# underactuated/HSLabs

Hardware: AMD Instinct MI355X
Metric: batched control-loop steps/sec (hexapod.xml, 18-DoF) at 1/2/4/8 MI355X (higher is better)
Workload: dtype f64

## Files before the change

### hslabs_amd/csrc/hs_limb.h

```cpp

#ifndef HS_LIMB_GROUP
#define HS_LIMB_GROUP HS_FUSED_GROUP
#endif
#ifndef HS_LIMB_WAVES
#define HS_LIMB_WAVES 2
#endif
#ifndef HS_LIMB_WAVES_F32
#define HS_LIMB_WAVES_F32 HS_LIMB_WAVES
#endif

constexpr int LG = 8;
constexpr int LGR = WAVE / LG;

__device__ unsigned long long g_limb_deferred;

template <int NM, bool FORCES = false>
struct LimbLds {
  real g[NM][6];
  real a[6];
  real wd[HS_NMAX];
  real p[FORCES ? NM : 1][3];
};

__device__ inline real grp_get(real v, int src) { return __shfl(v, src); }
// ... 29 lines not shown
  {
    const real cm[3] = {(real)lk.com[0], (real)lk.com[1], (real)lk.com[2]};
    mulp(H, cm, P);
  }
  {
    real R[9];
#pragma unroll
    for (int i = 0; i < 9; i++) R[i] = (real)lk.Rpj[i];
    auto a_rc = [&](int r, int c) { return H(r, 0) * R[c * 3 + 0] + H(r, 1) * R[c * 3 + 1] + H(r, 2) * R[c * 3 + 2]; };
    U[0] = (a_rc(2, 1) - a_rc(1, 2)) / 2;
    U[1] = (a_rc(0, 2) - a_rc(2, 0)) / 2;
    U[2] = (a_rc(1, 0) - a_rc(0, 1)) / 2;
  }
  if (CENTRE) {
#pragma unroll
    for (int i = 0; i < 3; i++) Jp[i] = Jv(i, 3);
#pragma unroll
    for (int i = 0; i < 3; i++) Jz[i] = Jv(i, 2);
    if (kk == 2) {
      const real cp[3] = {(real)lk.cap[0], (real)lk.cap[1], (real)lk.cap[2]};
      mulp(H, cp, fp);
      contact = fp[2] < (real)(T->rcap + 1e-4);
    }
  }
}

__device__ inline void part_dyn(real m, real inv, const real* Pm, const real* P0, const real* Pp, const real* Um,
                                const real* U0, const real* Up, real* f) {
  real vp[3], vm[3], mr[3], wp[3], wm[3], amr[3];
  for (int j = 0; j < 3; j++) {
    vp[j] = Pp[j] - P0[j];
    vp[j] *= inv;
    vm[j] = P0[j] - Pm[j];
    vm[j] *= inv;
    real mp = vp[j] * m, mm = vm[j] * m;
    mr[j] = mp - mm;
    mr[j] *= inv;
    wp[j] = Up[j] - U0[j];
    wp[j] *= inv;
    wm[j] = U0[j] - Um[j];
    wm[j] *= inv;
  }
  for (int j = 0; j < 3; j++) {
    amr[j] = wp[j] - wm[j];
    amr[j] *= inv;
  }
  for (int j = 0; j < 3; j++) {
    f[j] = mr[j];
    f[3 + j] = amr[j];
  }
  opaque_vals<6>(f);
  f[2] += m * real(1);
}

__device__ inline void part_g(const real* P, const real* o, real* f) {
  opaque_vals<6>(f);
  real d[3];
  for (int j = 0; j < 3; j++) d[j] = P[j] - o[j];
  f[3] += d[1] * f[2] - d[2] * f[1];
  f[4] += d[2] * f[0] - d[0] * f[2];
  f[5] += d[0] * f[1] - d[1] * f[0];
  opaque_vals<6>(f);
}

struct BodyS {
  real P[3], U[3];
};
__device__ inline BodyS body_straight(const real* bf, const real* u, real tv) {
  BodyS s;
  for (int i = 0; i < 3; i++) s.P[i] = fma(tv, u[i], bf[i]);
  for (int i = 0; i < 3; i++) s.U[i] = bf[3 + i];
  return s;
}
__device__ inline BodyS body_frame(const A34& A, const real* com) {
  BodyS s;
  mulp(A, com, s.P);
  s.U[0] = (A(2, 1) - A(1, 2)) / 2;
  s.U[1] = (A(0, 2) - A(2, 0)) / 2;
  s.U[2] = (A(1, 0) - A(0, 1)) / 2;
  return s;
}

__device__ __attribute__((always_inline)) inline A34 limb_frame(const hs_topo* T, int L, bool straight, const bool own,
                                                                const RolloutWS& W, int row, const real* u, real tv,
                                                                BodyS& ob) {
  if (straight) {
    if (own) ob = body_straight(W.kf.own[L][0], u, tv);
    return frame_at(load34r(W.kf.J0[L]), u, tv);
  }
  A34 A = load34r(W.ktor[row] + 6);
  const int clen = T->limb_chain_len[L];
  for (int kk = 1; kk < clen; kk++) {
    const int v = T->limb_chain[L][kk];
    A = mul(A, node_pj(T, v));
    if (T->node[v].owner_limb == L) {
      const real com[3] = {(real)T->node[v].com[0], (real)T->node[v].com[1], (real)T->node[v].com[2]};
      ob = body_frame(A, com);
    }
  }
  return mul(A, node_joint_parent(T, T->limb_child[L]));
}

__device__ inline bool sincos_big(real x) { return !(fabs(x) < (real)0x1p20); }
__device__ __attribute__((always_inline)) inline void limb_outer(const hs_topo* T, const hs_link (&LK)[3], const A34& J,
                                                                 const real* ja, real (&P)[3][3], real (&U)[3][3],
                                                                 bool& big) {
  real sq[3], cq[3];
#pragma unroll
  for (int kk = 0; kk < 3; kk++) {
    big |= sincos_big(ja[kk]);
    sincos_k_small(ja[kk], &sq[kk], &cq[kk]);
  }
  A34 Jv = J, H;
  real nul[3];
  bool nc = false;
#pragma unroll
  for (int kk = 0; kk < 3; kk++) fk_link<false>(T, LK[kk], kk, Jv, H, sq[kk], cq[kk], P[kk], U[kk], nul, nul, nul, nc);
}

__device__ __attribute__((always_inline)) inline void contact_block(const real (&Jp)[3][3], const real (&Jz)[3][3],
                                                                    const real (&xt)[3][3], const real* fp, real* Dp6,
                                                                    real* gc) {
  real tD[3][6], tg[3][3];
#pragma unroll
  for (int m = 0; m < 3; m++) {
    const int p = 2 - m;
    real Dp[6] = {0, 0, 0, 0, 0, 0}, g[3] = {0, 0, 0};
    real da[3], va[3][3];
    for (int r = 0; r < 3; r++) da[r] = Jp[p][r] - fp[r];
    cross_rows(da, va);
#pragma unroll
    for (int r = 0; r < 3; r++) {
      const real w2 = Jz[p][r] * Jz[p][r];
#pragma unroll
      for (int i = 0; i < 3; i++) {
        if (i == r) continue;
#pragma unroll
        for (int j = 0; j <= i; j++)
          if (j != r) Dp[i * (i + 1) / 2 + j] += w2 * va[r][i] * va[r][j];
        g[i] += w2 * va[r][i] * xt[p][r];
      }
    }
    for (int e = 0; e < 6; e++) tD[m][e] = Dp[e];
    for (int i = 0; i < 3; i++) tg[m][i] = g[i];
  }
#pragma unroll
  for (int e = 0; e < 6; e++) Dp6[e] = (tD[0][e] + tD[1][e]) + (tD[2][e] + real(0));
#pragma unroll
  for (int i = 0; i < 3; i++) gc[i] = (tg[0][i] + tg[1][i]) + (tg[2][i] + real(0));
}

template <int NM>
__device__ __attribute__((always_inline)) inline void limb_forces(const hs_topo* T, const hs_run_args& a,
                                                                  const hs::launch_map& mp, LimbLds<NM, true>& S, bool limb,
                                                                  int l, int L, int gbase, int nl, bool live, int b,
                                                                  int s_glob, const real* o,
                                                                  const real (&Jp)[3][3], const real (&Jz)[3][3],
                                                                  const real (&Pc)[3][3], const real* fp,
                                                                  const real (&xt)[3][3], bool bad, bool big) {
  const int n = T->n;
#ifdef HS_DBG
  const int dbg_r = live ? b * a.horizon + s_glob : -1;
#define FDBG(slot, val, n_)                                                                                      \
  do {                                                                                                           \
    if (HS_DBG == (n_) && dbg_r >= 0 && (size_t)dbg_r * 32 + (slot) < (1u << 22)) g_dbg[(size_t)dbg_r * 32 + (slot)] = (double)(val); \
  } while (0)
#else
#define FDBG(slot, val, n_) do {} while (0)
#endif
  real ts[9];
#pragma unroll
// ... 15 lines not shown
  const size_t orow = (size_t)b * a.horizon + s_glob;
  real Ct[18], Bd[6], Bl[9], rdB[3], rb[3], vl[27];
  bool okB = true;
  if (limb) {
    const real* z = inp(mp.tau_in) + (live ? orow : 0) * mp.st_tau;
    real zz[3];
    for (int kk = 0; kk < 3; kk++) zz[kk] = z[T->node[T->limb_node[L][kk]].hinge];
    ForcesRows F;
    forces_rows(F, Jp, Jz, Pc, fp, o, xt, zz);
    okB = forces_foot(F, fp, o, Ct, Bd, Bl, rdB, rb);
    FDBG(24 + dbg_f, Ct[0], 36);
    FDBG(24 + dbg_f, rb[0], 37);
    if (okB) {
      ForcesV G;
      forces_v(G, Ct, Bl, rdB, rb);
#pragma unroll
      for (int e = 0; e < 27; e++) {
        const TriWalk<> t(e < 21 ? e : 0);
        real pa = e < 21 ? F.prod(t.r, t.c) : F.prod(e - 21, 9);
        real pb = e < 21 ? G.vprod(t.r, t.c) : G.vprod(e - 21, 6);
        opaque_vals<1>(&pa);
        opaque_vals<1>(&pb);
        vl[e] = (e < 21) ? pb - pa : pb + pa;
      }
    }
  }
  const bool fast = !grp_any(limb && !okB, gbase);
  if (!fast || grp_any(big, gbase)) {
    if (l == 0 && live) {
      atomicAdd(&g_limb_deferred, 1ull);
      const int it = atomicAdd(mp.fix_count, 1);
      mp.fix_items[2 * it] = s_glob - mp.fused_s0;
      mp.fix_items[2 * it + 1] = b;
    }
    return;
  }
  real kv[27];
#pragma unroll
  for (int e = 0; e < 27; e++) {
    const real v = limb ? vl[e] : real(0);
    real s = real(0) + v;
    for (int k = 1; k < nl; k++) {
      const real prev = dpp_r<0x111>(s);
      if (l >= 1) s = prev + v;
    }
    const real tot = grp_get(s, gbase + nl - 1);
    const real dtv = (e < 21) ? real(0) : (e < 24 ? S.a[e - 21] : S.a[e - 21]);
    kv[e] = (e < 21) ? wtt_entry(e, ts, n) + tot : tot - dtv;
  }
  opaque_vals<27>(kv);
  if (l == 0) FDBG(1, kv[0], 33);
  real K[36], rd[6], lam[6];
#pragma unroll
  for (int r = 0; r < 6; r++) {
#pragma unroll
    for (int c = 0; c < 6; c++) K[6 * r + c] = (c <= r) ? kv[pk(r, c)] : real(0);
    lam[r] = kv[21 + r];
  }
  ldl_n<6>(K, real(0), rd);
  ldl_solve_n<6>(K, rd, lam);
  if (l == 0) FDBG(2, lam[0], 34);
  bool nan = false;
  real t[3] = {0, 0, 0};
  if (limb) {
    for (int k = 0; k < 3; k++) {
      real s = rb[k];
      for (int r = 0; r < 6; r++) s -= Ct[3 * r + k] * lam[r];
      t[k] = s;
    }
    ldl_solve_n<3>(Bl, rdB, t);
    FDBG(24 + dbg_f, t[0], 35);
    for (int k = 0; k < 3; k++) nan |= t[k] != t[k];
    const int f = T->link[L][2].foot;
    if (live && a.cf)
      for (int k = 0; k < 3; k++) outp(a.cf)[orow * mp.st_cf + 3 * f + k] = t[k];
  }
  if (live && a.cf)
    for (int c = 3 * T->nf + l; c < mp.st_cf; c += LG) outp(a.cf)[orow * mp.st_cf + c] = real(0);
  const bool any_nan = grp_any(nan, gbase), any_bad = grp_any(limb && bad, gbase);
  if (l == 0 && live && a.flags) a.flags[orow] = (any_nan ? HS_FLAG_NAN : 0u) | (any_bad ? HS_FLAG_UNREACH : 0u);
}
#undef FDBG


__device__ inline const limb_tile_entry& limb_tile_entry_of(const limb_tile_desc& d, int tile) { return d.tile[tile]; }
static_assert(HS_LMAX < LG, "lane LG - 1 of a group must not be a limb lane (lane_push's idle target)");
__device__ inline real lane_push(real v, int dst) {
  if constexpr (sizeof(real) == 8) {
    const double d = (double)v;
    const int lo = __builtin_amdgcn_ds_permute(dst << 2, __double2loint(d));
    const int hi = __builtin_amdgcn_ds_permute(dst << 2, __double2hiint(d));
    return (real)__hiloint2double(hi, lo);
  } else {
    return (real)__int_as_float(__builtin_amdgcn_ds_permute(dst << 2, __float_as_int((float)v)));
  }
}

#ifdef HS_DBG
#define TDBG(slot, val, n)                                                                                       \
  do {                                                                                                           \
    if (HS_DBG == (n) && dbg_r >= 0 && (size_t)dbg_r * 32 + (slot) < (1u << 22)) g_dbg[(size_t)dbg_r * 32 + (slot)] = (double)(val); \
  } while (0)
#else
#define TDBG(slot, val, n) do {} while (0)
#endif

#ifdef HS_STAMPS
#undef HS_STAMP_GATE
#define HS_STAMP_GATE stamp_on
#endif
template <bool FORCES>
__device__ __attribute__((always_inline)) inline void limb_tile_kd(
    const hs_topo* T_, real (&outer)[36][LGR * HS_LMAX], hs_link (&links)[HS_LMAX][3], const RolloutWS& W, bool straight,
    const real* u, real v, int lane, int nl, bool limb, int L, bool live, int row0, uint32_t M, uint64_t req,
    const real* tv, const real* o, real inv, real dt, real (&g3)[3][6], real (&Jp)[3][3], real (&Jz)[3][3], real* fp, bool& contact, bool& own,
    real* gown, real* jvel, real (&Pc)[3][3], real* Pown, bool& bad, bool& big, int dbg_r, bool stamp_on) {
  (void)dbg_r;
  (void)stamp_on;
  const int grp = lane >> 3, l = lane & 7;
  const bool shm = live && !((M >> (2 * grp)) & 1);
  const bool shp = live && !((M >> (2 * grp + 1)) & 1);
  const int nreq = __popc(M);
  auto nth_req = [req](int r) { return (int)(req >> (4 * r)) & 15; };
  const int nidle = LG - nl;
  const int E0 = (LGR * nidle) / nl;
  const int rqm = __popc(M & ((1u << (2 * grp)) - 1)), rqp = __popc(M & ((1u << (2 * grp + 1)) - 1));
  const int pm = shm || rqm < E0 ? 0 : 1 + (rqm - E0) / LGR, pp = shp || rqp < E0 ? 0 : 1 + (rqp - E0) / LGR;
  auto col = [](int ln) { return (ln >> 3) * HS_LMAX + (ln & 7); };
  real P[3][3], U[3][3];
  BodyS om, op, oc;
  own = limb && T_->limb_own_n[L] > 0;
  {
    int rq = 0, fL = L;
    bool extra = false;
    if (!limb) {
      const int j = grp * nidle + (l - nl);
      rq = j / nl;
      fL = j - rq * nl;
      extra = rq < E0 && rq < nreq;
      if (!extra) rq = 0, fL = 0;
    }
    const int bit = nth_req(rq), gr = bit >> 1, side = bit & 1;
    const int rr = __shfl(row0, gr * LG);
    const int frow = limb ? row0 + 2 : rr + 4 * side;
    const int dst = gr * LG + fL;
    const int dm = limb ? (shp ? lane + LG : -1) : (extra && side == 0 ? dst : -1);
    const int dp = limb ? (shm ? lane - LG : -1) : (extra && side == 1 ? dst : -1);
    BodyS ob;
#pragma unroll
    for (int j = 0; j < 3; j++) ob.P[j] = ob.U[j] = real(0);
    if (limb || extra) {
      const hs_topo* T = opaque_s(T_);
      const bool fown = T->limb_own_n[fL] > 0;
      const A34 J = limb_frame(T, fL, straight, fown, W, frow, u, W.t_tab[frow] * v, ob);
      const real* ja = W.ktab[frow][fL];
      real sq[3], cq[3];
#pragma unroll
      for (int kk = 0; kk < 3; kk++) sincos_k_small(ja[kk], &sq[kk], &cq[kk]);
      A34 Jv = J, H;
#pragma unroll
      for (int kk = 0; kk < 3; kk++)
        fk_link<true>(T, links[fL][kk], kk, Jv, H, sq[kk], cq[kk], P[kk], U[kk], Jp[kk], Jz[kk], fp, contact);
      if (dm >= 0) {
        const int c = col(dm);
#pragma unroll
        for (int kk = 0; kk < 3; kk++)
#pragma unroll
          for (int j = 0; j < 3; j++) {
            outer[3 * kk + j][c] = P[kk][j];
            outer[9 + 3 * kk + j][c] = U[kk][j];
          }
      }
      if (dp >= 0) {
        const int c = col(dp);
#pragma unroll
        for (int kk = 0; kk < 3; kk++)
#pragma unroll
          for (int j = 0; j < 3; j++) {
            outer[18 + 3 * kk + j][c] = P[kk][j];
            outer[27 + 3 * kk + j][c] = U[kk][j];
          }
      }
    }
    if (!limb) contact = false;
    oc = ob;
    if (!straight) {
#pragma unroll
      for (int j = 0; j < 6; j++) {
        const real val = j < 3 ? ob.P[j] : ob.U[j - 3];
        const real vm = lane_push(val, dm >= 0 ? dm : LG - 1), vp = lane_push(val, dp >= 0 ? dp : LG - 1);
        if (pm == 0) (j < 3 ? om.P[j] : om.U[j - 3]) = vm;
        if (pp == 0) (j < 3 ? op.P[j] : op.U[j - 3]) = vp;
      }
    }
  }
  STAMP(1);
  for (int base = E0, pass = 1; base < nreq; base += LGR, pass++) {
    const bool act = limb && base + grp < nreq;
    const int bit = nth_req(act ? base + grp : 0), gr = bit >> 1, side = bit & 1;
    const int frow = __shfl(row0, gr * LG) + 4 * side;
    const int dst = act ? gr * LG + L : -1;
    BodyS ob;
#pragma unroll
    for (int j = 0; j < 3; j++) ob.P[j] = ob.U[j] = real(0);
    __builtin_amdgcn_sched_barrier(0);
    if (act) {
      real P2[3][3], U2[3][3];
      bool nb = false;
      const hs_topo* T = opaque_s(T_);
      limb_outer(T, links[L], limb_frame(T, L, straight, own, W, frow, u, W.t_tab[frow] * v, ob), W.ktab[frow][L], P2, U2,
                 nb);
      const int c = col(dst), o0 = side ? 18 : 0;
#pragma unroll
      for (int kk = 0; kk < 3; kk++)
#pragma unroll
        for (int j = 0; j < 3; j++) {
          outer[o0 + 3 * kk + j][c] = P2[kk][j];
          outer[o0 + 9 + 3 * kk + j][c] = U2[kk][j];
        }
    }
    if (!straight) {
#pragma unroll
      for (int j = 0; j < 6; j++) {
        const real val = j < 3 ? ob.P[j] : ob.U[j - 3];
        const real vm = lane_push(val, act && side == 0 ? dst : LG - 1), vp = lane_push(val, act && side == 1 ? dst : LG - 1);
        if (pm == pass) (j < 3 ? om.P[j] : om.U[j - 3]) = vm;
        if (pp == pass) (j < 3 ? op.P[j] : op.U[j - 3]) = vp;
      }
    }
  }
  __builtin_amdgcn_sched_barrier(0);
  STAMP(2);
  wave_sync();
  if (limb) {
    const hs_topo* T = T_;
    if (own) {
      if (straight) {
        om = body_straight(W.kf.own[L][0], u, tv[0]);
        op = body_straight(W.kf.own[L][0], u, tv[4]);
      }
      part_dyn((real)T->mass[T->limb_own[L][0]], inv, om.P, oc.P, op.P, om.U, oc.U, op.U, gown);
      part_g(oc.P, o, gown);
      if constexpr (FORCES)
        for (int j = 0; j < 3; j++) Pown[j] = oc.P[j];
    }
    const int ol = grp * HS_LMAX + l;
#pragma unroll
    for (int kk = 0; kk < 3; kk++) {
      real* P0 = P[kk];
      real* U0 = U[kk];
      opaque_vals<3>(P0);
      if constexpr (FORCES)
        for (int j = 0; j < 3; j++) Pc[kk][j] = P0[j];
      opaque_vals<3>(U0);
      opaque_vals<3>(Jp[kk]);
      opaque_vals<3>(Jz[kk]);
      if (kk == 2) opaque_vals<3>(fp);
      real Pm[3], Um[3], Pp[3], Up[3];
#pragma unroll
      for (int j = 0; j < 3; j++) {
        Pm[j] = outer[3 * kk + j][ol];
        Um[j] = outer[9 + 3 * kk + j][ol];
        Pp[j] = outer[18 + 3 * kk + j][ol];
        Up[j] = outer[27 + 3 * kk + j][ol];
      }
      part_dyn((real)T->mass[T->limb_node[L][kk]], inv, Pm, P0, Pp, Um, U0, Up, g3[kk]);
      TDBG(T->limb_node[L][kk], P0[0], 1);
      TDBG(T->limb_node[L][kk], U0[0], 5);
      TDBG(T->limb_node[L][kk], g3[kk][0], 2);
      TDBG(T->limb_node[L][kk], g3[kk][3], 10);
      TDBG(T->limb_node[L][kk], g3[kk][1], 13);
      TDBG(T->limb_node[L][kk], g3[kk][2], 14);
      TDBG(T->limb_node[L][kk], g3[kk][4], 16);
      if (l == 0) TDBG(31, o[0], 15);
      if (l == 0) TDBG(30, o[1], 15);
      TDBG(T->limb_node[L][kk], Um[0], 9);
      TDBG(T->limb_node[L][kk], Up[0], 11);
      TDBG(T->limb_node[L][kk], Pm[0], 12);
      part_g(P0, o, g3[kk]);
      TDBG(T->limb_node[L][kk], g3[kk][3], 3);
    }
    bad = W.kbad[row0 + 2][L] != 0;
#pragma unroll
    for (int r = 0; r < 5; r += 2)
#pragma unroll
      for (int kk = 0; kk < 3; kk++) big |= sincos_big(W.ktab[row0 + r][L][kk]);
#pragma unroll
    for (int kk = 0; kk < 3; kk++) {
      if constexpr (FORCES) break;
      real dd = W.ktab[row0 + 3][L][kk] - W.ktab[row0 + 1][L][kk];
      if (dd > kPi) dd -= 2 * kPi;
      else if (dd < -kPi) dd += 2 * kPi;
      jvel[kk] = dd / (2 * dt);
    }
  }
}
#undef TDBG


template <int NM, bool FORCES, bool LOOP>
struct LimbShared {
  union {
    struct {
      real outer[36][LGR * HS_LMAX];
      hs_link links[HS_LMAX][3];
    } k;
    LimbLds<NM, FORCES> g[LGR];
  };
  __device__ hs_link (&links())[HS_LMAX][3] { return k.links; }
};
template <int NM, bool FORCES>
struct LimbShared<NM, FORCES, true> {
  union {
    struct {
      real outer[36][LGR * HS_LMAX];
    } k;
    LimbLds<NM, FORCES> g[LGR];
  };
  hs_link tl[HS_LMAX][3];
  __device__ hs_link (&links())[HS_LMAX][3] { return tl; }
};
static_assert(sizeof(LimbShared<HS_NMAX, false, true>) <= 20480, "a looping wavefront's LDS: 8 per CU's 160 KB");

struct LimbHead {
  int lane;
  int rslot, b;
  bool live;
  bool straight;
  const RolloutWS* W;
  real u[3];
};

template <class P>
__device__ inline const P* opaque_u(const P* p) {
  using cptr = const __attribute__((address_space(4))) P*;
  cptr q = (cptr)p;
  asm volatile("" : "+s"(q));
  return (const P*)q;
}

template <class P>
__device__ inline const P& opaque_k(const P& r) {
  using kptr = const __attribute__((address_space(4))) P*;
  kptr q = (kptr)&r;
  asm volatile("" : "+s"(q));
  return *(const P*)q;
}

template <int NM, bool FORCES, bool TILE, bool LOOP, class... PLAN>
__device__ __attribute__((always_inline)) inline void limb_step(LimbShared<NM, FORCES, LOOP>& sh, const hs_topo* __restrict__ T,
                                                                const hs_run_args& a0, const hs::launch_map& mp0,
                                                                const LimbHead& h, int fstep, bool stamp_on,
                                                                const PLAN&... plan) {
  (void)stamp_on;
  STAMP(23);
  int lane = h.lane;
  if constexpr (LOOP) {
    asm volatile("" : "+v"(lane));
    T = opaque_u(T);
  }
  const int grp = lane >> 3, l = lane & 7, gbase = lane & ~7, rslot = h.rslot, b = h.b;
  const int nl = T->n_limbs, nmj = T->nmj;
  const bool limb = l < nl, tlane = l == LG - 1, straight = h.straight;
  const int L = limb ? l : 0;
  const real u[3] = {h.u[0], h.u[1], h.u[2]};
  bool live = h.live;
  int tile_row = 0;
  uint32_t tile_M = 0;
  uint64_t tile_req = 0;
  if constexpr (TILE) {
    const limb_tile_entry& te = limb_tile_entry_of(plan..., fstep);
    const limb_tile_slot sl = te.slot[(unsigned)grp];
    live = sl.step >= 0;
    fstep = live ? sl.step : te.slot[0].step;
    tile_row = sl.row;
    tile_M = te.M;
    tile_req = te.req;
  }
  const RolloutWS* Wp = h.W;
  if constexpr (LOOP) Wp = opaque_u(Wp);
  const RolloutWS& W = *Wp;
  const real dt = W.st.dt;
  const real v = W.st.v;
  const real inv = real(1) / (2 * dt);
  LimbLds<NM, FORCES>& S = sh.g[grp];
  const int ol = grp * HS_LMAX + (l < HS_LMAX ? l : 0);
  const int s_glob = mp0.fused_s0 + fstep;
  int k0;
  if constexpr (TILE) {
    k0 = tile_row;
  } else {
    const int call = s_glob / mp0.fused_h;
    k0 = (int)(((int64_t)a0.k0 + (int64_t)call * mp0.fused_h) % a0.n_t) + s_glob % mp0.fused_h;
  }
  const int row0 = k0 - mp0.ktab_lo;
  real tv[5];
#pragma unroll
  for (int k = 0; k < 5; k += 2) tv[k] = W.t_tab[row0 + k] * v;
  real o[3];
  const real com0[3] = {(real)T->node[0].com[0], (real)T->node[0].com[1], (real)T->node[0].com[2]};
  if (straight) {
    for (int i = 0; i < 3; i++) o[i] = fma(tv[2], u[i], W.kf.torso[i]);
  } else {
    mulp(load34r(W.ktor[row0 + 2] + 6), com0, o);
  }
#ifdef HS_DBG
  const int dbg_r = live ? b * a0.horizon + s_glob : -1;
#define LDBG(slot, val, n)                                                                                       \
  do {                                                                                                           \
    if (HS_DBG == (n) && dbg_r >= 0 && (size_t)dbg_r * 32 + (slot) < (1u << 22)) g_dbg[(size_t)dbg_r * 32 + (slot)] = (double)(val); \
  } while (0)
#else
#define LDBG(slot, val, n) do {} while (0)
#endif

  real g0[6];
  {
    BodyS tb[3];
#pragma unroll
    for (int k = 0; k < 3; k++) {
      if (straight) tb[k] = body_straight(W.kf.torso, u, tv[2 * k]);
      else tb[k] = body_frame(load34r(W.ktor[row0 + 2 * k] + 6), com0);
    }
    part_dyn((real)T->mass[0], inv, tb[0].P, tb[1].P, tb[2].P, tb[0].U, tb[1].U, tb[2].U, g0);
    part_g(tb[1].P, o, g0);
  }
  STAMP(0);
  real g3[3][6];
  real Jp[3][3], Jz[3][3], fp[3];
  bool contact = false;
  bool own = false;
  real gown[6];
  real jvel[3];
  real Pc[3][3], Pown[3];
  bool bad = false, big = false;
  const hs_topo* const T_ = T;
  if constexpr (TILE) {
    limb_tile_kd<FORCES>(T_, sh.k.outer, sh.links(), W, straight, u, v, lane, nl, limb, L, live, row0, tile_M, tile_req, tv,
                         o, inv, dt, g3, Jp, Jz, fp, contact, own, gown, jvel, Pc, Pown, bad, big,
                         live ? b * a0.horizon + s_glob : -1, stamp_on);
  } else if (limb) {
    const int row = row0;
    own = T->limb_own_n[L] > 0;
    BodyS om, op, oc;
    {
      real P[3][3], U[3][3];
      const hs_topo* Ts = opaque_s(T);
      limb_outer(Ts, sh.k.links[L], limb_frame(Ts, L, straight, own, W, row, u, tv[0], om), W.ktab[row][L], P, U, big);
#pragma unroll
      for (int kk = 0; kk < 3; kk++)
#pragma unroll
        for (int j = 0; j < 3; j++) {
          sh.k.outer[3 * kk + j][ol] = P[kk][j];
          sh.k.outer[9 + 3 * kk + j][ol] = U[kk][j];
        }
    }
    STAMP(1);
    __builtin_amdgcn_sched_barrier(0);
    {
      real P[3][3], U[3][3];
      const hs_topo* Ts = opaque_s(T);
      limb_outer(Ts, sh.k.links[L], limb_frame(Ts, L, straight, own, W, row + 4, u, tv[4], op), W.ktab[row + 4][L], P, U,
                 big);
#pragma unroll
      for (int kk = 0; kk < 3; kk++)
#pragma unroll
        for (int j = 0; j < 3; j++) {
          sh.k.outer[18 + 3 * kk + j][ol] = P[kk][j];
          sh.k.outer[27 + 3 * kk + j][ol] = U[kk][j];
        }
    }
    __builtin_amdgcn_sched_barrier(0);
    STAMP(2);
    {
      const hs_topo* T = opaque_s(T_);
      const A34 J = limb_frame(T, L, straight, own, W, row + 2, u, tv[2], oc);
      if (own) {
        part_dyn((real)T->mass[T->limb_own[L][0]], inv, om.P, oc.P, op.P, om.U, oc.U, op.U, gown);
        part_g(oc.P, o, gown);
        if constexpr (FORCES)
          for (int j = 0; j < 3; j++) Pown[j] = oc.P[j];
      }
      const real* ja = W.ktab[row + 2][L];
      real sq[3], cq[3];
#pragma unroll
      for (int kk = 0; kk < 3; kk++) {
        big |= sincos_big(ja[kk]);
        sincos_k_small(ja[kk], &sq[kk], &cq[kk]);
      }
      A34 Jv = J, H;
#pragma unroll
      for (int kk = 0; kk < 3; kk++) {
        real P0[3], U0[3];
        fk_link<true>(T, sh.k.links[L][kk], kk, Jv, H, sq[kk], cq[kk], P0, U0, Jp[kk], Jz[kk], fp, contact);
        opaque_vals<3>(P0);
        if constexpr (FORCES)
          for (int j = 0; j < 3; j++) Pc[kk][j] = P0[j];
        opaque_vals<3>(U0);
        opaque_vals<3>(Jp[kk]);
        opaque_vals<3>(Jz[kk]);
        if (kk == 2) opaque_vals<3>(fp);
        real Pm[3], Um[3], Pp[3], Up[3];
        __builtin_amdgcn_sched_barrier(0);
#pragma unroll
        for (int j = 0; j < 3; j++) {
          Pm[j] = sh.k.outer[3 * kk + j][ol];
          Um[j] = sh.k.outer[9 + 3 * kk + j][ol];
          Pp[j] = sh.k.outer[18 + 3 * kk + j][ol];
          Up[j] = sh.k.outer[27 + 3 * kk + j][ol];
        }
        part_dyn((real)T->mass[T->limb_node[L][kk]], inv, Pm, P0, Pp, Um, U0, Up, g3[kk]);
        LDBG(T->limb_node[L][kk], P0[0], 1);
        LDBG(T->limb_node[L][kk], U0[0], 5);
        LDBG(T->limb_node[L][kk], g3[kk][0], 2);
        LDBG(T->limb_node[L][kk], g3[kk][3], 10);
        LDBG(T->limb_node[L][kk], g3[kk][1], 13);
        LDBG(T->limb_node[L][kk], g3[kk][2], 14);
        LDBG(T->limb_node[L][kk], g3[kk][4], 16);
        if (l == 0) LDBG(31, o[0], 15);
        if (l == 0) LDBG(30, o[1], 15);
        LDBG(T->limb_node[L][kk], Um[0], 9);
        LDBG(T->limb_node[L][kk], Up[0], 11);
        LDBG(T->limb_node[L][kk], Pm[0], 12);
        part_g(P0, o, g3[kk]);
        LDBG(T->limb_node[L][kk], g3[kk][3], 3);
      }
    }
    bad = W.kbad[row + 2][L] != 0;
#pragma unroll
    for (int kk = 0; kk < 3; kk++) {
      if constexpr (FORCES) break;
      real dd = W.ktab[row + 3][L][kk] - W.ktab[row + 1][L][kk];
      if (dd > kPi) dd -= 2 * kPi;
      else if (dd < -kPi) dd += 2 * kPi;
      jvel[kk] = dd / (2 * dt);
    }
  }
  STAMP(3);
  wave_sync();
  if (limb) {
#pragma unroll
    for (int kk = 0; kk < 3; kk++)
      for (int j = 0; j < 6; j++) S.g[T->limb_node[L][kk]][j] = g3[kk][j];
    if (own)
      for (int j = 0; j < 6; j++) S.g[T->limb_own[L][0]][j] = gown[j];
    if constexpr (FORCES) {
#pragma unroll
      for (int kk = 0; kk < 3; kk++)
        for (int j = 0; j < 3; j++) S.p[T->limb_node[L][kk]][j] = Pc[kk][j];
      if (own)
        for (int j = 0; j < 3; j++) S.p[T->limb_own[L][0]][j] = Pown[j];
    }
  } else if (tlane) {
    for (int j = 0; j < 6; j++) S.g[0][j] = g0[j];
  }
  wave_sync();

  STAMP(4);
  real xt[3][3];
  if (limb) {
#pragma unroll
    for (int kk = 0; kk < 3; kk++) {
      real F[3] = {0, 0, 0}, V[3] = {0, 0, 0};
#pragma unroll
      for (int m = kk; m < 3; m++)
        for (int j = 0; j < 3; j++) { F[j] += g3[m][j]; V[j] += g3[m][3 + j]; }
      opaque_vals<3>(F);
      opaque_vals<3>(V);
      real d[3];
      for (int j = 0; j < 3; j++) d[j] = Jp[kk][j] - o[j];
      V[0] -= d[1] * F[2] - d[2] * F[1];
      V[1] -= d[2] * F[0] - d[0] * F[2];
      V[2] -= d[0] * F[1] - d[1] * F[0];
      for (int j = 0; j < 3; j++) xt[kk][j] = V[j];
      opaque_vals<3>(xt[kk]);
      LDBG(T->limb_node[L][kk], V[0], 4);
      LDBG(T->limb_node[L][kk], F[0], 18);
      LDBG(T->limb_node[L][kk], d[0], 17);
    }
  }
  {
    const int nk = T->node[0].nkids;
    if (l < nk && l < HS_CMAX) {
      const int c = T->node[0].kids[l], sz = T->node[c].size;
      real Fk[3] = {0, 0, 0}, Vk[3] = {0, 0, 0};
#pragma unroll
      for (int r = 0; r < 8; r++)
        if (r < sz)
          for (int j = 0; j < 3; j++) { Fk[j] += S.g[c + r][j]; Vk[j] += S.g[c + r][3 + j]; }
      for (int r = 8; r < sz; r++)
        for (int j = 0; j < 3; j++) { Fk[j] += S.g[c + r][j]; Vk[j] += S.g[c + r][3 + j]; }
      for (int j = 0; j < 3; j++) { S.g[c][j] = Fk[j]; S.g[c][3 + j] = Vk[j]; }
    }
  }
  wave_sync();
  if (tlane) {
    real F[3], V[3];
    for (int j = 0; j < 3; j++) { F[j] = S.g[0][j]; V[j] = S.g[0][3 + j]; }
    const int nk = T->node[0].nkids;
    for (int kk = 0; kk < HS_CMAX; kk++) {
      if (kk >= nk) break;
      const int c = T->node[0].kids[kk];
      for (int j = 0; j < 3; j++) { F[j] += S.g[c][j]; V[j] += S.g[c][3 + j]; }
    }
    const real d[3] = {0, 0, 0};
    V[0] -= d[1] * F[2] - d[2] * F[1];
    V[1] -= d[2] * F[0] - d[0] * F[2];
    V[2] -= d[0] * F[1] - d[1] * F[0];
    for (int j = 0; j < 3; j++) { S.a[j] = F[j]; S.a[3 + j] = V[j]; }
  }
  wave_sync();

  STAMP(5);
  const hs_run_args& a = LOOP ? opaque_k(a0) : a0;
  const hs::launch_map& mp = LOOP ? opaque_k(mp0) : mp0;
  if constexpr (FORCES) {
    limb_forces<NM>(T, a, mp, S, limb, l, L, gbase, nl, live, b, s_glob, o, Jp, Jz, Pc, fp, xt, bad, big);
    return;
  }
  const int fiL = T->link[L][2].foot;
  const uint32_t cm = grp_or((limb && contact) ? 1u << fiL : 0u);
  const int nc = __popc(cm);
  const bool mine = limb && contact;
  if (limb) LDBG(24 + fiL, fp[2], 25);
  int src = 0;
  for (int L2 = 0; L2 < nl; L2++) {
    const int f2 = T->link[L2][2].foot;
    if (((cm >> f2) & 1) && __popc(cm & ((1u << f2) - 1)) == l) src = L2;
  }
  src += gbase;
  const bool slot = l < nc;
  bool defer = grp_any(big, gbase);
  bool nearf = false;
  real y3[3] = {0, 0, 0};
  real d0[3] = {0, 0, 0}, Dinv[9], gc[3], Dp6[6];
  if (mine)
    for (int r = 0; r < 3; r++) d0[r] = o[r] - fp[r];
  if (mine && nc >= 2) contact_block(Jp, Jz, xt, fp, Dp6, gc);
  if (nc >= 3) {
    float e0 = grp_getf(float(o[0] - fp[0]), src), e1 = grp_getf(float(o[1] - fp[1]), src),
          e2 = grp_getf(float(o[2] - fp[2]), src);
    if (!slot) e0 = e1 = e2 = 0.f;
    {
      const float s0 = group8_sum(e0), s1 = group8_sum(e1), s2 = group8_sum(e2);
      const float q00 = group8_sum(e0 * e0), q11 = group8_sum(e1 * e1), q22 = group8_sum(e2 * e2);
      const float q01 = group8_sum(e0 * e1), q02 = group8_sum(e0 * e2), q12 = group8_sum(e1 * e2);
      const float k = float(nc);
      const float c00 = k * q00 - s0 * s0, c11 = k * q11 - s1 * s1, c22 = k * q22 - s2 * s2;
      const float c01 = k * q01 - s0 * s1, c02 = k * q02 - s0 * s2, c12 = k * q12 - s1 * s2;
      const float c2 = (c00 * c11 - c01 * c01) + (c00 * c22 - c02 * c02) + (c11 * c22 - c12 * c12);
      const float tq = q00 + q11 + q22;
      const float md = fmaxf(k, fmaxf(tq - q00, fmaxf(tq - q11, tq - q22)));
      const float t = kZerothGuard * k * (c00 + c11 + c22) * md;
      const bool well = c2 >= t;
      const bool nearz = c2 >= t / float(kNearBand) && c2 <= t * float(kNearBand);
      defer |= !well;
      nearf |= nearz;
    }
    STAMP(6);
    real sch[27];
#pragma unroll
    for (int e = 0; e < 27; e++) sch[e] = 0;
    bool lnear = false, ok = true;
    if (mine) {
      const real* Dp = Dp6;
      opaque_vals<3>(d0);
      const real D[9] = {Dp[0], Dp[1], Dp[3], Dp[1], Dp[2], Dp[4], Dp[3], Dp[4], Dp[5]};
      LDBG(24 + fiL, Dp[0], 6);
      LDBG(24 + fiL, gc[0], 7);
      real Lm[9];
      for (int i = 0; i < 9; i++) Lm[i] = D[i];
      real rl[3];
      ok = ldl_n<3>(Lm, kFastPivotGuard, rl, lnear);
      if (ok) {
        for (int j = 0; j < 3; j++) {
          real e[3] = {0, 0, 0};
          e[j] = 1;
          ldl_solve_n<3>(Lm, rl, e);
          for (int i = 0; i < 3; i++) Dinv[3 * i + j] = e[i];
        }
#pragma unroll
        for (int r = 0; r < 6; r++) {
          real E[3];
#pragma unroll
          for (int j = 0; j < 3; j++) {
            real acc = 0;
#pragma unroll
            for (int i = 0; i < 3; i++) acc += a_entry(d0, r, i) * Dinv[3 * i + j];
            E[j] = acc;
          }
#pragma unroll
          for (int qq = 0; qq <= r; qq++) {
            real vv = 0;
#pragma unroll
            for (int j = 0; j < 3; j++) vv += E[j] * a_entry(d0, qq, j);
            sch[sch_lower(r, qq)] = vv;
          }
          real hh = 0;
          for (int j = 0; j < 3; j++) hh += E[j] * gc[j];
          sch[SCH_H + r] = hh;
        }
      }
    }
// ... 87 lines not shown
        gg[0][r] = grp_get(gc[r], s0);
        gg[1][r] = grp_get(gc[r], s1);
      }
      for (int e = 0; e < 6; e++) {
        Dc[0][e] = grp_get(Dp6[e], s0);
        Dc[1][e] = grp_get(Dp6[e], s1);
      }
      const real Dm[2][9] = {{Dc[0][0], Dc[0][1], Dc[0][3], Dc[0][1], Dc[0][2], Dc[0][4], Dc[0][3], Dc[0][4], Dc[0][5]},
                             {Dc[1][0], Dc[1][1], Dc[1][3], Dc[1][1], Dc[1][2], Dc[1][4], Dc[1][3], Dc[1][4], Dc[1][5]}};
      real u[3], un = 0;
      for (int r = 0; r < 3; r++) { u[r] = f0[r] - f1[r]; un += u[r] * u[r]; }
      un = sqrt(un);
      ok = un > real(1e-12);
      real nv[6], M[36], bv[6], rl[6];
      if (ok) {
        for (int r = 0; r < 3; r++) { nv[r] = u[r] / un / sqrt(real(2)); nv[3 + r] = -nv[r]; }
        const bool first = mine && __popc(cm & ((1u << fiL) - 1)) == 0;
        if (first) LDBG(24 + fiL, nv[2], 26);
        for (int i = 0; i < 6; i++) {
          const real* di = dA[i / 3];
          for (int j = 0; j < 6; j++) {
            const real* dj = dA[j / 3];
            real sv = 0;
            for (int r = 0; r < 6; r++) sv += a_entry(di, r, i % 3) * a_entry(dj, r, j % 3);
            M[6 * i + j] = sv + nv[i] * nv[j];
          }
          real sv = 0;
          for (int r = 0; r < 6; r++) sv += a_entry(di, r, i % 3) * a[r];
          bv[i] = -sv;
        }
        if (first) LDBG(24 + fiL, M[5], 27);
        opaque_vals<36>(M);
        opaque_vals<6>(bv);
        opaque_vals<6>(nv);
        ok = chol_n<6>(M, kFastPivotGuard, rl, lnear);
      }
      if (ok) {
        chol_solve_n<6>(M, rl, bv);
        opaque_vals<6>(bv);
        real nDn = 0, nr = 0;
        for (int c = 0; c < 2; c++)
          for (int i = 0; i < 3; i++) {
            real Dw = 0, Dn = 0;
            for (int j = 0; j < 3; j++) { Dw += Dm[c][3 * i + j] * bv[3 * c + j]; Dn += Dm[c][3 * i + j] * nv[3 * c + j]; }
            nr += nv[3 * c + i] * (Dw + gg[c][i]);
            nDn += nv[3 * c + i] * Dn;
          }
        ok = nDn > 0;
        if (ok) {
          real t = -nr / nDn;
          for (int i = 0; i < 6; i++) y[i] = bv[i] + t * nv[i];
          if (mine && __popc(cm & ((1u << fiL) - 1)) == 0) {
            LDBG(24 + fiL, y[0], 22);
            LDBG(24 + fiL, bv[0], 23);
            LDBG(24 + fiL, t, 24);
          }
        }
      }
    }
    defer |= !ok;
    nearf |= lnear;
    if (mine && ok) {
      const int rk = __popc(cm & ((1u << fiL) - 1));
      for (int i = 0; i < 3; i++) y3[i] = rk == 0 ? y[i] : y[3 + i];
      opaque_vals<3>(y3);
    }
  }
  STAMP(8);
  if (defer) {
    if (l == 0 && live) {
      atomicAdd(&g_limb_deferred, 1ull);
      const int it = atomicAdd(mp.fix_count, 1);
      mp.fix_items[2 * it] = s_glob - mp.fused_s0;
      mp.fix_items[2 * it + 1] = mp.limb_slots ? mp.limb_slots[rslot] : b;
    }
    return;
  }

  const size_t orow = (size_t)b * a.horizon + s_glob;
  bool nan = false;
  if (limb) {
#pragma unroll
    for (int kk = 0; kk < 3; kk++) {
      const int hh = T->link[L][kk].hinge;
      real d[3], yy[3];
#pragma unroll
      for (int rr = 0; rr < 3; rr++) {
        d[rr] = Jp[kk][rr] - fp[rr];
        yy[rr] = mine ? y3[rr] : real(0);
      }
      real tq = real(0);
#pragma unroll
      for (int r = 0; r < 3; r++) {
        real s = real(0);
#pragma unroll
        for (int jj = 0; jj < 3; jj++)
          if (jj != r) s = s + cross_e(d, jj, r) * yy[jj];
        real xr = xt[kk][r] + s;
        tq = tq + Jz[kk][r] * xr;
      }
      real dw = tq * jvel[kk];
      S.wd[hh] = (dw > 0) ? dw : 0;
      nan |= tq != tq;
      if (live && a.tau) outp(a.tau)[orow * mp.st_tau + hh] = tq;
    }
    if (mine)
      for (int j = 0; j < 3; j++) nan |= y3[j] != y3[j];
    if (live && a.cf)
      for (int j = 0; j < 3; j++) {
        real zv = -real(0);
        if (mine) zv = -(real(0) + (real(-1)) * y3[j]);
        outp(a.cf)[orow * mp.st_cf + 3 * fiL + j] = zv;
      }
  }
  if (live && mp.limb_rollouts) {
    if (a.tau)
      for (int c = nmj + l; c < mp.st_tau; c += LG) outp(a.tau)[orow * mp.st_tau + c] = real(0);
    if (a.cf)
      for (int c = 3 * T->nf + l; c < mp.st_cf; c += LG) outp(a.cf)[orow * mp.st_cf + c] = real(0);
  }
  const bool any_nan = grp_any(nan, gbase), any_bad = grp_any(limb && bad, gbase);
  wave_sync();
  if (l == 0 && live) {
    uint32_t flags = 0;
    if (nc == 0) flags |= HS_FLAG_NO_CONTACT;
    if (nc == 1) flags |= HS_FLAG_FULL_RANK;
    if (nearf) flags |= HS_FLAG_NEAR_RANK;
    if (any_nan) flags |= HS_FLAG_NAN;
    if (any_bad) flags |= HS_FLAG_UNREACH;
    if (a.flags) a.flags[orow] = flags;
    real work_dt = real(0);
    for (int jj = 0; jj < nmj; jj++) work_dt += S.wd[jj];
    reinterpret_cast<real*>(mp.fused_work)[(size_t)s_glob * a.n_rollouts + b] = work_dt;
  }
  STAMP(9);
  RSTAMP(17);
}
#undef LDBG
#ifdef HS_STAMPS
#undef HS_STAMP_GATE
#define HS_STAMP_GATE true
#endif

struct LimbTileArgs {
  const hs_topo* T0;
  hs_run_args a;
  RolloutWS* rws;
  hs::launch_map mp;
  limb_tile_desc plan;
};

template <int NM, bool FORCES, bool TILE = false, class... PLAN>
__global__ __launch_bounds__(WAVE, HS_REAL_IS_FLOAT ? HS_LIMB_WAVES_F32 : HS_LIMB_WAVES) void hs_limb_kernel(const hs_topo* __restrict__ T0, hs_run_args a,
                                                                      RolloutWS* __restrict__ rws, hs::launch_map mp, PLAN... plan) {
  static_assert(sizeof...(PLAN) == (TILE ? 1 : 0), "the tile mapping takes the launch's tile descriptor, the packed mapping nothing");
  static_assert(!TILE || (std::is_same<PLAN, limb_tile_desc>::value && ...), "LimbTileArgs holds a limb_tile_desc");
  static_assert(offsetof(LimbTileArgs, a) == 8 && offsetof(LimbTileArgs, rws) == 8 + sizeof(hs_run_args) &&
                    offsetof(LimbTileArgs, mp) == 16 + sizeof(hs_run_args) &&
                    offsetof(LimbTileArgs, plan) == 16 + sizeof(hs_run_args) + sizeof(hs::launch_map) &&
                    alignof(hs_run_args) == 8 && alignof(hs::launch_map) == 8,
                "LimbTileArgs: the kernel argument segment packs the arguments in order at their alignment");
  constexpr bool LOOP = TILE && !FORCES && !HS_REAL_IS_FLOAT;
  __shared__ LimbShared<NM, FORCES, LOOP> sh;
  int fstep = 0, q = (int)blockIdx.x;
  const int nt = TILE ? limb_tile_count(mp.fused_n) : 0, tl = LOOP ? mp.limb_tile_loop : 1;
  fused_coords<HS_LIMB_GROUP>((int)blockIdx.x, mp.fused_w, TILE ? HS_TILE_SLOTS * limb_tile_chunks(nt, tl) : mp.fused_n, fstep,
                              q);
  const hs_topo* __restrict__ T = mp.limb_model ? T0 + mp.limb_model[q] : T0;
  {
    const uint64_t* src = reinterpret_cast<const uint64_t*>(&T->link[0][0]);
    uint64_t* dst = reinterpret_cast<uint64_t*>(&sh.links()[0][0]);
    constexpr int NW = sizeof(hs_link[HS_LMAX][3]) / sizeof(uint64_t);
    for (int e = (int)threadIdx.x; e < NW; e += WAVE) dst[e] = src[e];
    wave_sync();
  }
  RSTAMP(16);
  STAMP(15);
  LimbHead h;
  h.lane = (int)threadIdx.x;
  h.rslot = q * LGR + (TILE ? fstep % LGR : h.lane >> 3);
  h.b = mp.limb_rollouts ? mp.limb_rollouts[h.rslot] : h.rslot;
  h.live = h.b >= 0 && h.b < a.n_rollouts;
  if (TILE && !h.live) return;
  const int bb = h.live ? h.b : (mp.limb_rollouts ? mp.limb_rollouts[q * LGR] : a.n_rollouts - 1);
  h.W = &rws[bb];
  const hs_gait_params& gp = a.params[bb];
  h.straight = (real)gp.curvature == 0 && !gp.rec_transform_flag;
  {
    const NodeK n0 = load_nodek(T, 0);
    for (int i = 0; i < 3; i++) h.u[i] = n0.Jp(i, 0);
  }
  if constexpr (LOOP) {
    const int c = fstep / LGR;
    for (int t0 = limb_tile_chunk_first(c, tl), t = t0, te = limb_tile_chunk_end(c, tl, nt); t < te; t++) {
      using kptr = const __attribute__((address_space(4))) LimbTileArgs*;
      kptr ka = (kptr)__builtin_amdgcn_kernarg_segment_ptr();
      asm volatile("" : "+s"(ka));
      const LimbTileArgs& k = *(const LimbTileArgs*)ka;
#ifdef HS_STAMPS
      const bool stamp_on = t - t0 == g_stamp_iter;
#else
      const bool stamp_on = true;
#endif
      limb_step<NM, FORCES, true, true>(sh, T, k.a, k.mp, h, t, stamp_on, k.plan);
      wave_sync();
    }
  } else {
    limb_step<NM, FORCES, TILE, false>(sh, T, a, mp, h, TILE ? fstep / LGR : fstep, true, plan...);
  }
}
```

Measured before the change: 1.025 billion.

## Stage per-limb topology constants and rollout time/frame tables in LDS for looping limb kernel

In the looping tile path, the kernel now precomputes compact per-limb records (masses, node, hinge and foot indices, root kid info) and copies the rollout's t_tab and kinematic frames into shared memory once per wavefront. Inner-loop steps read these from LDS instead of chasing hs_topo and RolloutWS through global memory. The tile slot word is selected with register selects rather than an indexed load, and the joint-velocity and big-angle checks use batched ktab loads. The cost is extra LDS per wavefront, which may lower occupancy, plus a one-time copy at kernel start.

```diff
diff --git a/hslabs_amd/csrc/hs_limb.h b/hslabs_amd/csrc/hs_limb.h
--- a/hslabs_amd/csrc/hs_limb.h
+++ b/hslabs_amd/csrc/hs_limb.h
@@ -135,11 +135,11 @@
 }
 
 __device__ __attribute__((always_inline)) inline A34 limb_frame(const hs_topo* T, int L, bool straight, const bool own,
-                                                                const RolloutWS& W, int row, const real* u, real tv,
-                                                                BodyS& ob) {
+                                                                const RolloutWS& W, const KinFrames& kf, int row,
+                                                                const real* u, real tv, BodyS& ob) {
   if (straight) {
-    if (own) ob = body_straight(W.kf.own[L][0], u, tv);
-    return frame_at(load34r(W.kf.J0[L]), u, tv);
+    if (own) ob = body_straight(kf.own[L][0], u, tv);
+    return frame_at(load34r(kf.J0[L]), u, tv);
   }
   A34 A = load34r(W.ktor[row] + 6);
   const int clen = T->limb_chain_len[L];
@@ -321,6 +321,64 @@
 }
 #undef FDBG
 
+struct LimbLaneK {
+  real m[3], mown;
+  uint32_t nodes;
+  uint32_t hf;
+  uint32_t kid;
+  uint32_t pad_;
+};
+static_assert(HS_NMAX < 256 && HS_LMAX < 256, "LimbLaneK packs node, hinge and foot indices into bytes");
+struct LimbRolloutK {
+  real t_tab[HS_KTAB];
+  KinFrames kf;
+};
+static_assert(offsetof(RolloutWS, kf) == offsetof(RolloutWS, t_tab) + sizeof(real[HS_KTAB]) &&
+                  offsetof(LimbRolloutK, kf) == sizeof(real[HS_KTAB]),
+              "LimbRolloutK mirrors RolloutWS from t_tab through kf");
+
+template <bool LOOP>
+struct LimbModelK {
+  const hs_topo* T;
+  const LimbLaneK* k;
+  __device__ bool own(int L) const {
+    if constexpr (LOOP) return (k[L].kid >> 16) & 1;
+    else return T->limb_own_n[L] > 0;
+  }
+  __device__ int node(int L, int kk) const {
+    if constexpr (LOOP) return (k[L].nodes >> (8 * kk)) & 255;
+    else return T->limb_node[L][kk];
+  }
+  __device__ int own_node(int L) const {
+    if constexpr (LOOP) return k[L].nodes >> 24;
+    else return T->limb_own[L][0];
+  }
+  __device__ real mass(int L, int kk) const {
+    if constexpr (LOOP) return k[L].m[kk];
+    else return (real)T->mass[T->limb_node[L][kk]];
+  }
+  __device__ real mass_own(int L) const {
+    if constexpr (LOOP) return k[L].mown;
+    else return (real)T->mass[T->limb_own[L][0]];
+  }
+  __device__ int hinge(int L, int kk) const {
+    if constexpr (LOOP) return (k[L].hf >> (8 * kk)) & 255;
+    else return T->link[L][kk].hinge;
+  }
+  __device__ int foot(int L) const {
+    if constexpr (LOOP) return k[L].hf >> 24;
+    else return T->link[L][2].foot;
+  }
+  __device__ int kid(int l) const {
+    if constexpr (LOOP) return k[l].kid & 255;
+    else return T->node[0].kids[l];
+  }
+  __device__ int kid_size(int l, int c) const {
+    if constexpr (LOOP) return (k[l].kid >> 8) & 255;
+    else return T->node[c].size;
+  }
+};
+
 
 __device__ inline const limb_tile_entry& limb_tile_entry_of(const limb_tile_desc& d, int tile) { return d.tile[tile]; }
 static_assert(HS_LMAX < LG, "lane LG - 1 of a group must not be a limb lane (lane_push's idle target)");
@@ -348,9 +406,10 @@
 #undef HS_STAMP_GATE
 #define HS_STAMP_GATE stamp_on
 #endif
-template <bool FORCES>
+template <bool FORCES, bool LOOP>
 __device__ __attribute__((always_inline)) inline void limb_tile_kd(
-    const hs_topo* T_, real (&outer)[36][LGR * HS_LMAX], hs_link (&links)[HS_LMAX][3], const RolloutWS& W, bool straight,
+    const hs_topo* T_, const LimbModelK<LOOP>& mk, const KinFrames& kf, const real* ttab,
+    real (&outer)[36][LGR * HS_LMAX], hs_link (&links)[HS_LMAX][3], const RolloutWS& W, bool straight,
     const real* u, real v, int lane, int nl, bool limb, int L, bool live, int row0, uint32_t M, uint64_t req,
     const real* tv, const real* o, real inv, real dt, real (&g3)[3][6], real (&Jp)[3][3], real (&Jz)[3][3], real* fp, bool& contact, bool& own,
     real* gown, real* jvel, real (&Pc)[3][3], real* Pown, bool& bad, bool& big, int dbg_r, bool stamp_on) {
@@ -368,7 +427,7 @@
   auto col = [](int ln) { return (ln >> 3) * HS_LMAX + (ln & 7); };
   real P[3][3], U[3][3];
   BodyS om, op, oc;
-  own = limb && T_->limb_own_n[L] > 0;
+  own = limb && mk.own(L);
   {
     int rq = 0, fL = L;
     bool extra = false;
@@ -390,8 +449,9 @@
     for (int j = 0; j < 3; j++) ob.P[j] = ob.U[j] = real(0);
     if (limb || extra) {
       const hs_topo* T = opaque_s(T_);
-      const bool fown = T->limb_own_n[fL] > 0;
-      const A34 J = limb_frame(T, fL, straight, fown, W, frow, u, W.t_tab[frow] * v, ob);
+      const bool fown = LimbModelK<LOOP>{T, mk.k}.own(fL);
+      const real tvf = LOOP && limb ? tv[2] : ttab[frow] * v;
+      const A34 J = limb_frame(T, fL, straight, fown, W, kf, frow, u, tvf, ob);
       const real* ja = W.ktab[frow][fL];
       real sq[3], cq[3];
 #pragma unroll
@@ -447,8 +507,8 @@
       real P2[3][3], U2[3][3];
       bool nb = false;
       const hs_topo* T = opaque_s(T_);
-      limb_outer(T, links[L], limb_frame(T, L, straight, own, W, frow, u, W.t_tab[frow] * v, ob), W.ktab[frow][L], P2, U2,
-                 nb);
+      limb_outer(T, links[L], limb_frame(T, L, straight, own, W, kf, frow, u, ttab[frow] * v, ob), W.ktab[frow][L], P2,
+                 U2, nb);
       const int c = col(dst), o0 = side ? 18 : 0;
 #pragma unroll
       for (int kk = 0; kk < 3; kk++)
@@ -473,12 +533,13 @@
   wave_sync();
   if (limb) {
     const hs_topo* T = T_;
+    (void)T;
     if (own) {
       if (straight) {
-        om = body_straight(W.kf.own[L][0], u, tv[0]);
-        op = body_straight(W.kf.own[L][0], u, tv[4]);
-      }
-      part_dyn((real)T->mass[T->limb_own[L][0]], inv, om.P, oc.P, op.P, om.U, oc.U, op.U, gown);
+        om = body_straight(kf.own[L][0], u, tv[0]);
+        op = body_straight(kf.own[L][0], u, tv[4]);
+      }
+      part_dyn(mk.mass_own(L), inv, om.P, oc.P, op.P, om.U, oc.U, op.U, gown);
       part_g(oc.P, o, gown);
       if constexpr (FORCES)
         for (int j = 0; j < 3; j++) Pown[j] = oc.P[j];
@@ -503,7 +564,7 @@
         Pp[j] = outer[18 + 3 * kk + j][ol];
         Up[j] = outer[27 + 3 * kk + j][ol];
       }
-      part_dyn((real)T->mass[T->limb_node[L][kk]], inv, Pm, P0, Pp, Um, U0, Up, g3[kk]);
+      part_dyn(mk.mass(L, kk), inv, Pm, P0, Pp, Um, U0, Up, g3[kk]);
       TDBG(T->limb_node[L][kk], P0[0], 1);
       TDBG(T->limb_node[L][kk], U0[0], 5);
       TDBG(T->limb_node[L][kk], g3[kk][0], 2);
@@ -520,6 +581,24 @@
       TDBG(T->limb_node[L][kk], g3[kk][3], 3);
     }
     bad = W.kbad[row0 + 2][L] != 0;
+    if constexpr (LOOP) {
+      real jq[5][3];
+#pragma unroll
+      for (int r = 0; r < 5; r++)
+#pragma unroll
+        for (int kk = 0; kk < 3; kk++) jq[r][kk] = W.ktab[row0 + r][L][kk];
+#pragma unroll
+      for (int r = 0; r < 5; r += 2)
+#pragma unroll
+        for (int kk = 0; kk < 3; kk++) big |= sincos_big(jq[r][kk]);
+#pragma unroll
+      for (int kk = 0; kk < 3; kk++) {
+        const real dd = jq[3][kk] - jq[1][kk];
+        const real lo = dd - 2 * kPi, hi = dd + 2 * kPi;
+        jvel[kk] = (dd > kPi ? lo : (dd < -kPi ? hi : dd)) / (2 * dt);
+      }
+      return;
+    }
 #pragma unroll
     for (int r = 0; r < 5; r += 2)
 #pragma unroll
@@ -557,6 +636,8 @@
     LimbLds<NM, FORCES> g[LGR];
   };
   hs_link tl[HS_LMAX][3];
+  LimbRolloutK rk;
+  LimbLaneK lk[LG];
   __device__ hs_link (&links())[HS_LMAX][3] { return tl; }
 };
 static_assert(sizeof(LimbShared<HS_NMAX, false, true>) <= 20480, "a looping wavefront's LDS: 8 per CU's 160 KB");
@@ -609,9 +690,24 @@
   uint64_t tile_req = 0;
   if constexpr (TILE) {
     const limb_tile_entry& te = limb_tile_entry_of(plan..., fstep);
-    const limb_tile_slot sl = te.slot[(unsigned)grp];
+    limb_tile_slot sl;
+    int first;
+    if constexpr (LOOP) {
+      static_assert(sizeof(limb_tile_slot) == 4 && HS_TILE_SLOTS == 8, "a slot is one word: step low, row high");
+      uint32_t w[HS_TILE_SLOTS];
+      __builtin_memcpy(w, te.slot, sizeof(w));
+      uint32_t ws = w[0];
+#pragma unroll
+      for (int g = 1; g < HS_TILE_SLOTS; g++) ws = grp == g ? w[g] : ws;
+      sl.step = (int16_t)(ws & 0xFFFFu);
+      sl.row = (int16_t)(ws >> 16);
+      first = (int16_t)(w[0] & 0xFFFFu);
+    } else {
+      sl = te.slot[(unsigned)grp];
+      first = te.slot[0].step;
+    }
     live = sl.step >= 0;
-    fstep = live ? sl.step : te.slot[0].step;
+    fstep = live ? sl.step : first;
     tile_row = sl.row;
     tile_M = te.M;
     tile_req = te.req;
@@ -633,9 +729,20 @@
     k0 = (int)(((int64_t)a0.k0 + (int64_t)call * mp0.fused_h) % a0.n_t) + s_glob % mp0.fused_h;
   }
   const int row0 = k0 - mp0.ktab_lo;
+  const real* ttab;
+  const KinFrames* kfp;
+  LimbModelK<LOOP> mk{T, nullptr};
+  if constexpr (LOOP) {
+    ttab = sh.rk.t_tab;
+    kfp = &sh.rk.kf;
+    mk.k = sh.lk;
+  } else {
+    ttab = W.t_tab;
+    kfp = &W.kf;
+  }
   real tv[5];
 #pragma unroll
-  for (int k = 0; k < 5; k += 2) tv[k] = W.t_tab[row0 + k] * v;
+  for (int k = 0; k < 5; k += 2) tv[k] = ttab[row0 + k] * v;
   real o[3];
   const real com0[3] = {(real)T->node[0].com[0], (real)T->node[0].com[1], (real)T->node[0].com[2]};
   if (straight) {
@@ -675,7 +782,7 @@
   bool bad = false, big = false;
   const hs_topo* const T_ = T;
   if constexpr (TILE) {
-    limb_tile_kd<FORCES>(T_, sh.k.outer, sh.links(), W, straight, u, v, lane, nl, limb, L, live, row0, tile_M, tile_req, tv,
+    limb_tile_kd<FORCES, LOOP>(T_, mk, *kfp, ttab, sh.k.outer, sh.links(), W, straight, u, v, lane, nl, limb, L, live, row0, tile_M, tile_req, tv,
                          o, inv, dt, g3, Jp, Jz, fp, contact, own, gown, jvel, Pc, Pown, bad, big,
                          live ? b * a0.horizon + s_glob : -1, stamp_on);
   } else if (limb) {
@@ -685,7 +792,7 @@
     {
       real P[3][3], U[3][3];
       const hs_topo* Ts = opaque_s(T);
-      limb_outer(Ts, sh.k.links[L], limb_frame(Ts, L, straight, own, W, row, u, tv[0], om), W.ktab[row][L], P, U, big);
+      limb_outer(Ts, sh.k.links[L], limb_frame(Ts, L, straight, own, W, W.kf, row, u, tv[0], om), W.ktab[row][L], P, U, big);
 #pragma unroll
       for (int kk = 0; kk < 3; kk++)
 #pragma unroll
@@ -699,7 +806,7 @@
     {
       real P[3][3], U[3][3];
       const hs_topo* Ts = opaque_s(T);
-      limb_outer(Ts, sh.k.links[L], limb_frame(Ts, L, straight, own, W, row + 4, u, tv[4], op), W.ktab[row + 4][L], P, U,
+      limb_outer(Ts, sh.k.links[L], limb_frame(Ts, L, straight, own, W, W.kf, row + 4, u, tv[4], op), W.ktab[row + 4][L], P, U,
                  big);
 #pragma unroll
       for (int kk = 0; kk < 3; kk++)
@@ -713,7 +820,7 @@
     STAMP(2);
     {
       const hs_topo* T = opaque_s(T_);
-      const A34 J = limb_frame(T, L, straight, own, W, row + 2, u, tv[2], oc);
+      const A34 J = limb_frame(T, L, straight, own, W, W.kf, row + 2, u, tv[2], oc);
       if (own) {
         part_dyn((real)T->mass[T->limb_own[L][0]], inv, om.P, oc.P, op.P, om.U, oc.U, op.U, gown);
         part_g(oc.P, o, gown);
@@ -780,15 +887,15 @@
   if (limb) {
 #pragma unroll
     for (int kk = 0; kk < 3; kk++)
-      for (int j = 0; j < 6; j++) S.g[T->limb_node[L][kk]][j] = g3[kk][j];
+      for (int j = 0; j < 6; j++) S.g[mk.node(L, kk)][j] = g3[kk][j];
     if (own)
-      for (int j = 0; j < 6; j++) S.g[T->limb_own[L][0]][j] = gown[j];
+      for (int j = 0; j < 6; j++) S.g[mk.own_node(L)][j] = gown[j];
     if constexpr (FORCES) {
 #pragma unroll
       for (int kk = 0; kk < 3; kk++)
-        for (int j = 0; j < 3; j++) S.p[T->limb_node[L][kk]][j] = Pc[kk][j];
+        for (int j = 0; j < 3; j++) S.p[mk.node(L, kk)][j] = Pc[kk][j];
       if (own)
-        for (int j = 0; j < 3; j++) S.p[T->limb_own[L][0]][j] = Pown[j];
+        for (int j = 0; j < 3; j++) S.p[mk.own_node(L)][j] = Pown[j];
     }
   } else if (tlane) {
     for (int j = 0; j < 6; j++) S.g[0][j] = g0[j];
@@ -821,7 +928,7 @@
   {
     const int nk = T->node[0].nkids;
     if (l < nk && l < HS_CMAX) {
-      const int c = T->node[0].kids[l], sz = T->node[c].size;
+      const int c = mk.kid(l), sz = mk.kid_size(l, c);
       real Fk[3] = {0, 0, 0}, Vk[3] = {0, 0, 0};
 #pragma unroll
       for (int r = 0; r < 8; r++)
@@ -857,7 +964,7 @@
     limb_forces<NM>(T, a, mp, S, limb, l, L, gbase, nl, live, b, s_glob, o, Jp, Jz, Pc, fp, xt, bad, big);
     return;
   }
-  const int fiL = T->link[L][2].foot;
+  const int fiL = mk.foot(L);
   const uint32_t cm = grp_or((limb && contact) ? 1u << fiL : 0u);
   const int nc = __popc(cm);
   const bool mine = limb && contact;
@@ -1111,7 +1218,7 @@
   if (limb) {
 #pragma unroll
     for (int kk = 0; kk < 3; kk++) {
-      const int hh = T->link[L][kk].hinge;
+      const int hh = mk.hinge(L, kk);
       real d[3], yy[3];
 #pragma unroll
       for (int rr = 0; rr < 3; rr++) {
@@ -1196,12 +1303,42 @@
   fused_coords<HS_LIMB_GROUP>((int)blockIdx.x, mp.fused_w, TILE ? HS_TILE_SLOTS * limb_tile_chunks(nt, tl) : mp.fused_n, fstep,
                               q);
   const hs_topo* __restrict__ T = mp.limb_model ? T0 + mp.limb_model[q] : T0;
+  STAMP(18);
   {
     const uint64_t* src = reinterpret_cast<const uint64_t*>(&T->link[0][0]);
     uint64_t* dst = reinterpret_cast<uint64_t*>(&sh.links()[0][0]);
     constexpr int NW = sizeof(hs_link[HS_LMAX][3]) / sizeof(uint64_t);
     for (int e = (int)threadIdx.x; e < NW; e += WAVE) dst[e] = src[e];
-    wave_sync();
+    if constexpr (LOOP) {
+      const int l = (int)threadIdx.x;
+      if (l < LG) {
+        LimbLaneK e;
+        e.m[0] = e.m[1] = e.m[2] = e.mown = real(0);
+        e.nodes = e.hf = e.kid = e.pad_ = 0;
+        if (l < T->n_limbs) {
+          const bool own = T->limb_own_n[l] > 0;
+          const int on = own ? T->limb_own[l][0] : 0;
+#pragma unroll
+          for (int kk = 0; kk < 3; kk++) {
+            const int v = T->limb_node[l][kk];
+            e.m[kk] = (real)T->mass[v];
+            e.nodes |= (uint32_t)v << (8 * kk);
+            e.hf |= (uint32_t)T->link[l][kk].hinge << (8 * kk);
+          }
+          if (own) e.mown = (real)T->mass[on];
+          e.nodes |= (uint32_t)on << 24;
+          e.hf |= (uint32_t)T->link[l][2].foot << 24;
+          e.kid = (uint32_t)own << 16;
+        }
+        if (l < T->node[0].nkids && l < HS_CMAX) {
+          const int c = T->node[0].kids[l];
+          e.kid |= (uint32_t)c | (uint32_t)T->node[c].size << 8;
+        }
+        sh.lk[l] = e;
+      }
+    } else {
+      wave_sync();
+    }
   }
   RSTAMP(16);
   STAMP(15);
@@ -1220,6 +1357,13 @@
     for (int i = 0; i < 3; i++) h.u[i] = n0.Jp(i, 0);
   }
   if constexpr (LOOP) {
+    {
+      const real* src = h.W->t_tab;
+      real* dst = sh.rk.t_tab;
+      constexpr int NR = sizeof(LimbRolloutK) / sizeof(real);
+      for (int e = (int)threadIdx.x; e < NR; e += WAVE) dst[e] = src[e];
+      wave_sync();
+    }
     const int c = fstep / LGR;
     for (int t0 = limb_tile_chunk_first(c, tl), t = t0, te = limb_tile_chunk_end(c, tl, nt); t < te; t++) {
       using kptr = const __attribute__((address_space(4))) LimbTileArgs*;
```

Result: faster. 1.082 billion (median of 6 runs) (+5.5%).
